# peterbudai/redux

Hardware: AMD Instinct MI355X
Metric: encode MB/s (whole node), per-block bitstream bit-exact (higher is better)
Workload: dtype u32

## Files before the change

### redux_amd/csrc/redux_hip.hip

```cpp
#include "redux_coder.hpp"
#include "redux_any.hpp"
#include "redux_gen.hpp"
#include "redux_encode.hpp"
#include "redux_decode.hpp"
#include "redux_decode_adaptive.hpp"
#include "redux_decode_wave.hpp"
#include "redux_decode_cells.hpp"
#include "redux_pack.hpp"
#include "redux_table.hpp"
#include "redux_coop.hpp"
#include "redux_synth.hpp"
#include "redux_static.hpp"
#include "redux_planes.hpp"
#include "redux_delta.hpp"
#include "redux_base.hpp"
#include "redux_hist.hpp"
#include "redux_plane_static.hpp"
#include "redux_segment_static.hpp"
#include "redux_context_static.hpp"
#include "redux_crc.hpp"
#include "redux_store.hpp"
#include "redux_const.hpp"
#include "redux_cost.hpp"

// ... 38 lines not shown
    const int st = any::compress_stream(P, a.trees + blk * a.tree_words, a.in + o0, len, a.slots + blk * a.slot_bytes,
                                        a.slot_cap, bi, bo);
    a.sizes[blk]  = (uint32_t)bo;
    a.status[blk] = st;
}

struct AnyDecArgs {
    const uint8_t  *in;
    const uint64_t *in_offsets;
    uint64_t        nblocks;
    uint8_t        *out;
    uint32_t       *out_sizes;
    int32_t        *status;
    uint64_t       *in_used;
    uint32_t       *trees;
    uint64_t        tree_words;
    uint32_t        block_size;
    uint32_t        sb, fb, cb;
};

__global__ void __launch_bounds__(64) k_decode_any(AnyDecArgs a)
{
    const uint64_t blk = (uint64_t)blockIdx.x * 64 + threadIdx.x;
    if (blk >= a.nblocks)
        return;
    const uint64_t o0 = a.in_offsets[blk], o1 = a.in_offsets[blk + 1];
    const any::Params P = any::make_params(a.sb, a.fb, a.cb);
    uint64_t  bi, bo;
    const int st = any::decompress_stream(P, a.trees + blk * a.tree_words, a.in + o0, o1 - o0,
                                          a.out + blk * (uint64_t)a.block_size, a.block_size, bi, bo);
    a.out_sizes[blk] = (uint32_t)bo;
    a.status[blk]    = st;
    if (a.in_used)
        a.in_used[blk] = bi;
}

static inline uint64_t align_up(uint64_t v, uint64_t a) { return (v + a - 1) / a * a; }

struct Geometry {
    uint64_t nblocks;
    uint64_t slot_bytes;
    uint32_t slot_cap;
    uint32_t rc_n;
    uint32_t nfreeze;
    bool     u16, fixup;
    bool     any;
    bool     gen;
    uint64_t tree_bytes;
    bool     coop;
    bool     coop_linear;
    uint32_t pair_width;
    uint32_t coop_win;
    uint32_t coop_nwin;
    uint64_t off_rc, off_sizes, off_mode, off_slots, off_trees, off_table, off_seen, off_cstate, off_pairs, total;
};

static int check_params(const redux_params *p)
{
    if (!p)
        return REDUX_INVALID_INPUT;
    const int st = redux_params_check(p->symbol_bits, p->freq_bits, p->code_bits);
    if (st != REDUX_OK)
        return st;
    if (p->symbol_bits > 16)
        return REDUX_UNSUPPORTED;
    return REDUX_OK;
}

static bool is_any(const redux_params *p) { return p->symbol_bits != 8 || p->code_bits > 32; }
static uint64_t gen_updates(const redux_params *p, uint32_t block_size)
{
    const uint64_t nsym    = (uint64_t)block_size * 8 / p->symbol_bits;
    const uint64_t nfreeze = ((1ull << p->freq_bits) - 1) - ((1ull << p->symbol_bits) + 1);
    return nsym < nfreeze ? nsym : nfreeze;
}
static bool gen_decode_cells(const redux_params *p, uint32_t block_size)
{
    if (p->symbol_bits >= 8)
        return gen_updates(p, block_size) + (1ull << (p->symbol_bits - 1)) <= 65535;
    return true;
}
static bool gen_needs_fixup(const redux_params *p, uint32_t block_size)
{
    return p->symbol_bits < 8 && (1ull << p->symbol_bits) + 1 + gen_updates(p, block_size) > (1ull << 17) + 64;
}
static bool is_gen(const redux_params *p, uint32_t block_size)
{
    if (p->code_bits > 32 || p->symbol_bits == 8 || p->symbol_bits > 12 || block_size > (1u << 22))
        return false;
    return gen_decode_cells(p, block_size);
}
static bool gen_decode_in_workspace(const redux_params *p, uint64_t nblocks)
{
    (void)nblocks;
    return p->symbol_bits >= 11;
}
static uint64_t gen_decode_tree_bytes(const redux_params *p) { return (1ull << (p->symbol_bits - 4)) * 32; }
static bool cells8_takes(const redux_params *p, uint32_t block_size, uint64_t nslots, bool table)
{
    return p->symbol_bits == 8 && p->code_bits <= 32 && block_size > 65536 && block_size <= (1u << 22) &&
           (nslots == 0 || nslots > kWaveDecMaxBlocks || (nslots > kWaveDecManyBlocks && block_size >= kWaveDecLargeBlock)) && !table;
}
static uint32_t cells8_rc_entries(const redux_params *p, uint32_t block_size)
{
    const uint64_t nfreeze = ((1ull << p->freq_bits) - 1) - 257;
    return (uint32_t)((block_size < nfreeze ? block_size : nfreeze) + 1 + 32);
}
static bool cells8_needs_fixup(const redux_params *p, uint32_t block_size)
{
    return 257ull + cells8_rc_entries(p, block_size) - 33 > (1ull << 17) + 64;
}

static uint64_t slot_cap_for(const redux_params *p, uint32_t block_size)
{
    const uint64_t freq_max = (1ull << p->freq_bits) - 1;
    if (is_any(p)) {
        const uint64_t K = (1ull << p->symbol_bits) + 1;
        const uint64_t n = (uint64_t)block_size * 8 / p->symbol_bits + 1;
        uint32_t       lg = 0;
        while ((1ull << lg) < K + n)
            lg++;
        const uint64_t per = (lg < p->freq_bits ? lg : p->freq_bits) + 2;
        return n * per / 8 + p->code_bits / 8 + 64;
    }
    const uint64_t n        = block_size;
    const bool     freezes  = 257ull + n > freq_max;
    const uint64_t bits     = freezes ? n * (p->freq_bits + 2) : n * 9;
    return bits / 8 + 1024;
}

static Geometry geometry(const redux_params *p, uint64_t in_len, uint32_t block_size, bool static_model = false, bool allow_coop = true)
{
    Geometry g;
    memset(&g, 0, sizeof g);
    g.nblocks = in_len == 0 ? 1 : (in_len + block_size - 1) / block_size;
    const uint64_t cap = static_model ? ((uint64_t)block_size + 1) * (p->freq_bits + 2) / 8 + 1024 : slot_cap_for(p, block_size);
    g.slot_cap   = cap > 0xFFFFFF00ull ? 0xFFFFFF00u : (uint32_t)cap;
    g.slot_bytes = align_up((uint64_t)g.slot_cap + 32, 128);
    if (((g.slot_bytes / 128) & 1) == 0)
        g.slot_bytes += 128;
    const uint64_t freq_max = (1ull << p->freq_bits) - 1;
    g.nfreeze = (uint32_t)(freq_max - 257);
    const uint64_t maxlen = in_len < block_size ? in_len : block_size;
    g.rc_n  = (uint32_t)((maxlen < g.nfreeze ? maxlen : g.nfreeze) + 1);
    g.u16   = block_size <= 65536;
    g.fixup = (257ull + (uint64_t)(g.rc_n - 1)) >= (1ull << 17);
    g.rc_n += 32;
    g.any = !static_model && is_any(p);
    if (static_model)
        g.rc_n = 0;
    g.gen = !static_model && is_gen(p, block_size) && 64ull * g.slot_bytes < (1ull << 32);
    if (g.gen) {
        const uint64_t k0      = (1ull << p->symbol_bits) + 1;
        const uint64_t nsym    = maxlen * 8 / p->symbol_bits;
        const uint64_t nfreeze = freq_max - k0;
        g.any     = false;
        g.nfreeze = (uint32_t)(nfreeze < 0xFFFFFFFFull ? nfreeze : 0xFFFFFFFFull);
        g.rc_n    = (uint32_t)((nsym < nfreeze ? nsym : nfreeze) + 1 + 32);
        g.u16     = false;
        g.fixup   = true;
        g.tree_bytes = 0;
    }
    if (g.any) {
        g.rc_n       = 0;
        g.u16        = false;
        g.fixup      = true;
        g.tree_bytes = align_up(((1ull << p->symbol_bits) + 2) * 4, 256);
    }
    g.pair_width = g.u16 ? 64u : 1u;
    const uint64_t lanes_total = g.u16 ? (g.nblocks + 63) / 64 * 64 : g.nblocks;
    g.coop_win  = block_size + 1;
    g.coop_nwin = 1;
    if (!g.u16) {
        uint64_t w = kCoopWindowBytes / 2 / (8 * lanes_total);
        w = w > kCoopWindowMax ? kCoopWindowMax : w;
        w = w < 4096 ? 4096 : w;
        if (w < (uint64_t)block_size + 1) {
            g.coop_nwin = (uint32_t)(((uint64_t)block_size + 1 + w - 1) / w);
            g.coop_win  = (uint32_t)((((uint64_t)block_size + 1 + g.coop_nwin - 1) / g.coop_nwin + 31) & ~31ull);
        }
    }
    const uint64_t pair_bytes = (g.u16 ? lanes_total * ((uint64_t)g.coop_win + kCoopSlack) : 2 * lanes_total * coop_block_pitch(g.coop_win)) * 8;
    const bool linear = g.nblocks < 64 && !g.u16;
    g.coop = allow_coop && !static_model && !g.any && !g.gen && g.nblocks <= (g.u16 ? kCoopMaxBlocks : kCoopMaxLargeBlocks) && block_size >= kCoopMinBlock &&
             (linear ? g.nblocks : 64ull) * g.slot_bytes < (1ull << 32) && pair_bytes <= (g.u16 ? kCoopMaxPairBytes : kCoopWindowBytes + (64ull << 20));
    if (g.coop)
        g.rc_n = g.u16 ? g.coop_win + 64 : 2 * ((g.coop_win + 64 + 31) & ~31u);
    g.coop_linear = g.coop && linear;
    g.off_rc    = 0;
    g.off_sizes = align_up(g.off_rc + (uint64_t)g.rc_n * 8, 256);
    g.off_mode  = align_up(g.off_sizes + g.nblocks * 4, 256);
    g.off_slots = g.off_mode + 256 + kClaimWords * 4;
    const bool     one_each = g.coop_linear || (!g.any && !g.gen && !static_model && !g.coop && 64ull * g.slot_bytes >= (1ull << 32));
    const uint64_t nslots = one_each ? g.nblocks : (g.nblocks + 63) / 64 * 64 + 1;
    g.off_trees = align_up(g.off_slots + nslots * g.slot_bytes + (g.nblocks + 63) / 64 * 128, 256);
    g.off_table = align_up(g.off_trees + (g.gen ? (g.nblocks + 63) / 64 * 64 : g.nblocks) * g.tree_bytes, 256);
    g.off_seen  = g.off_table + align_up(g.nblocks * sizeof(redux_block), 256);
    g.off_cstate = g.off_seen + align_up(table_seen_words(g.nblocks) * 4, 256);
    g.off_pairs  = g.off_cstate + ((g.coop && !g.u16) ? align_up(g.nblocks * (8 + 256) * 4, 256) : 0);
    g.total = g.off_pairs + (g.coop ? pair_bytes : 0);
    return g;
}

static Geometry geometry_ws(const redux_params *p, uint64_t in_len, uint32_t block_size, uint64_t workspace_bytes)
{
    Geometry g = geometry(p, in_len, block_size);
    if (g.coop && workspace_bytes < g.total)
        g = geometry(p, in_len, block_size, false, false);
    return g;
}

#define HIP_TRY(expr)                                                                                  \
    do {                                                                                               \
        hipError_t e_ = (expr);                                                                        \
        if (e_ != hipSuccess) {                                                                        \
            fprintf(stderr, "redux_hip: %s failed: %s (%s:%d)\n", #expr, hipGetErrorString(e_),       \
                    __FILE__, __LINE__);                                                               \
            return REDUX_IO_ERROR;                                                                     \
        }                                                                                              \
    } while (0)

static uint32_t cu_count()
{
    static std::atomic<int> cus[16];
    int dev = 0;
    if (hipGetDevice(&dev) != hipSuccess || dev < 0 || dev >= 16)
        return 256;
    int n = cus[dev].load(std::memory_order_relaxed);
    if (n == 0) {
        if (hipDeviceGetAttribute(&n, hipDeviceAttributeMultiprocessorCount, dev) != hipSuccess || n <= 0)
            n = 256;
        cus[dev].store(n, std::memory_order_relaxed);
    }
    return (uint32_t)n;
}

enum class EncKernel { PairCb32, Pair, SingleU16, SingleU32, Gen, GenPair, Any, CoopCb32, Coop };
enum class DecKernel { LockCb32, Lock, GenericU16, GenericU32, Cells, CellsFixup, CellsWorkspace, Cells8, Cells8Fixup, Any, Wave, WaveFixup };

static uint32_t encode_lanes(const Geometry &g, uint32_t block_size)
{
    return (64ull * g.slot_bytes < (1ull << 32) && 64ull * block_size < (1ull << 32)) ? 64u : 1u;
}

static EncKernel pick_encode_kernel(const Geometry &g, const redux_params *p, bool aligned16, uint32_t block_size)
{
    if (g.gen)
        return p->symbol_bits < 8 ? EncKernel::Gen : EncKernel::GenPair;
    if (g.any)
        return EncKernel::Any;
    bool coop = g.coop;
#ifdef REDUX_AB
    if (getenv("REDUX_ENCODE_KERNEL"))
        coop = false;
#endif
    if (coop)
        return p->code_bits == 32 ? EncKernel::CoopCb32 : EncKernel::Coop;
    bool pair = g.u16 && aligned16 && encode_lanes(g, block_size) == 64;
#ifdef REDUX_AB
    const char *force = getenv("REDUX_ENCODE_KERNEL");
    if (force && !strcmp(force, "single"))
        pair = false;
#endif
    if (pair)
        return p->code_bits == 32 ? EncKernel::PairCb32 : EncKernel::Pair;
    return g.u16 ? EncKernel::SingleU16 : EncKernel::SingleU32;
}

static Geometry decode_geometry(const redux_params *p, uint32_t block_size) { return geometry(p, block_size, block_size, false, false); }

static DecKernel pick_decode_kernel(const Geometry &g, const redux_params *p, uint64_t nslots, uint32_t block_size, bool table)
{
    if (g.gen) {
        if (gen_needs_fixup(p, block_size))
            return DecKernel::CellsFixup;
        return gen_decode_in_workspace(p, nslots ? nslots : ~0ull) ? DecKernel::CellsWorkspace : DecKernel::Cells;
    }
    if (g.any)
        return DecKernel::Any;
    if (cells8_takes(p, block_size, nslots, table))
        return cells8_needs_fixup(p, block_size) ? DecKernel::Cells8Fixup : DecKernel::Cells8;
    bool wave = nslots != 0 && nslots <= kWaveDecMaxBlocks && !(g.u16 && !g.fixup);
#ifdef REDUX_AB
    if (getenv("REDUX_DECODE_KERNEL"))
        wave = false;
#endif
    if (wave)
        return g.fixup ? DecKernel::WaveFixup : DecKernel::Wave;
    bool lock = g.u16 && !g.fixup;
#ifdef REDUX_AB
    if (getenv("REDUX_DECODE_KERNEL"))
        lock = false;
#endif
    if (lock)
        return p->code_bits == 32 ? DecKernel::LockCb32 : DecKernel::Lock;
    return g.u16 ? DecKernel::GenericU16 : DecKernel::GenericU32;
}

}

#include "redux_host.hpp"

using namespace redux;

static host::EncodeCoder adaptive_encoder(const redux_params *p, uint32_t block_size)
{
    return {[=](uint64_t max_in, bool several, uint64_t &ws, uint64_t &bound) {
                ws    = several ? geometry(p, max_in, block_size, false, false).total : redux_encode_workspace_bytes(p, max_in, block_size);
                bound = redux_encode_bound(p, max_in, block_size);
            },
            [=](host::Slot &s, uint64_t len, uint64_t bound, void *ws, uint64_t ws_bytes, hipStream_t st) {
                return redux_encode_blocks_dev(p, s.d_in.p, len, block_size, s.d_out.p, bound, s.d_off.p, s.d_st.p, s.d_sum.p, ws,
                                               ws_bytes, st);
            }};
}

static host::EncodeCoder static_encoder(const redux_params *p, const uint32_t *cum, uint32_t block_size)
{
    return {[=](uint64_t max_in, bool, uint64_t &ws, uint64_t &bound) {
// ... 396 lines not shown
}

uint64_t redux_encode_bound(const redux_params *p, uint64_t in_len, uint32_t block_size)
{
    if (check_params(p) != REDUX_OK || block_size == 0)
        return 0;
    const Geometry g = geometry(p, in_len, block_size);
    return g.nblocks * (uint64_t)g.slot_cap;
}

uint64_t redux_encode_workspace_bytes(const redux_params *p, uint64_t in_len, uint32_t block_size)
{
    if (check_params(p) != REDUX_OK || block_size == 0)
        return 0;
    return geometry(p, in_len, block_size).total;
}

static int encode_slots_impl(const redux_params *p, const void *d_in, uint64_t in_len, uint32_t block_size,
                             const redux_block *d_table, uint64_t tbl_blocks, bool tbl_aligned16, void *d_block_status,
                             void *d_workspace, uint64_t workspace_bytes, void *stream, uint64_t nblocks_real = 0)
{
    int st = check_params(p);
    if (st != REDUX_OK)
        return st;
    if (block_size == 0 || !d_workspace || !d_block_status || (in_len && !d_in))
        return REDUX_INVALID_INPUT;
    const Geometry g = geometry_ws(p, d_table ? tbl_blocks * (uint64_t)block_size : in_len, block_size, workspace_bytes);
    if (d_table && (g.gen || g.any || in_len > 0xFFFFFFFFull || tbl_blocks == 0))
        return tbl_blocks == 0 ? REDUX_INVALID_INPUT : REDUX_UNSUPPORTED;
    if (workspace_bytes < g.total)
        return REDUX_OUTPUT_TOO_SMALL;
    if (((uintptr_t)d_workspace) & 255)
        return REDUX_INVALID_INPUT;
    hipStream_t s  = (hipStream_t)stream;
    uint8_t    *ws = (uint8_t *)d_workspace;

    if (d_table) {
        TableCheckArgs ta;
        ta.in         = d_table;
        ta.out        = (redux_block *)(ws + g.off_table);
        ta.nentries   = tbl_blocks;
        ta.nblocks    = nblocks_real;
        ta.bytes      = in_len;
        ta.block_size = block_size;
        ta.aligned16  = tbl_aligned16 ? 1u : 0u;
        ta.seen       = (uint32_t *)(ws + g.off_seen);
        ta.sizes      = (uint32_t *)(ws + g.off_sizes);
        ta.status     = (int32_t *)d_block_status;
        const uint64_t n0 = std::max(nblocks_real, table_seen_words(nblocks_real));
        k_table_prepare<<<(uint32_t)((n0 + 255) / 256), 256, 0, s>>>(ta);
        k_table_check<<<(uint32_t)((tbl_blocks + 255) / 256), 256, 0, s>>>(ta);
        d_table = ta.out;
    }
    HIP_TRY(hipMemsetAsync(ws + g.off_mode, 0, 256 + kClaimWords * 4, s));
    if (g.gen) {
        GenEncArgs ga;
        ga.in         = (const uint8_t *)d_in;
        ga.in_len     = in_len;
        ga.nblocks    = g.nblocks;
        ga.slots      = ws + g.off_slots;
        ga.slot_bytes = g.slot_bytes;
        ga.sizes      = (uint32_t *)(ws + g.off_sizes);
        ga.status     = (int32_t *)d_block_status;
        ga.rc         = (const double *)(ws + g.off_rc);
        ga.block_size = block_size;
        ga.slot_cap   = g.slot_cap;
        ga.nfreeze    = g.nfreeze;
        ga.code_bits  = p->code_bits;
        k_fill_rc_from<<<(g.rc_n + 255) / 256, 256, 0, s>>>((double *)(ws + g.off_rc), g.rc_n, (1u << p->symbol_bits) + 1u);
        const uint32_t grid64 = (uint32_t)((g.nblocks + 63) / 64);
        switch (p->symbol_bits) {
#define REDUX_GEN_ENC(SB) case SB: k_encode_gen<SB><<<grid64, 64, 0, s>>>(ga); break;
#define REDUX_GEN_ENC_PAIR(SB)                                                                                         \
    case SB: k_encode_gen_pair<SB><<<(uint32_t)((g.nblocks + GenTree<SB>::kBlocks - 1) / GenTree<SB>::kBlocks), 256, 0, s>>>(ga); break;
            REDUX_GEN_ENC(1) REDUX_GEN_ENC(2) REDUX_GEN_ENC(3) REDUX_GEN_ENC(4) REDUX_GEN_ENC(5) REDUX_GEN_ENC(6) REDUX_GEN_ENC(7)
            REDUX_GEN_ENC_PAIR(9) REDUX_GEN_ENC_PAIR(10) REDUX_GEN_ENC_PAIR(11) REDUX_GEN_ENC_PAIR(12)
#undef REDUX_GEN_ENC
#undef REDUX_GEN_ENC_PAIR
        default: return REDUX_UNSUPPORTED;
        }
        HIP_TRY(hipGetLastError());
        return REDUX_OK;
    }
    if (g.any) {
        AnyEncArgs aa;
        aa.in         = (const uint8_t *)d_in;
        aa.in_len     = in_len;
        aa.nblocks    = g.nblocks;
        aa.slots      = ws + g.off_slots;
        aa.slot_bytes = g.slot_bytes;
        aa.sizes      = (uint32_t *)(ws + g.off_sizes);
        aa.status     = (int32_t *)d_block_status;
        aa.trees      = (uint32_t *)(ws + g.off_trees);
        aa.tree_words = g.tree_bytes / 4;
        aa.block_size = block_size;
        aa.slot_cap   = g.slot_cap;
        aa.sb = p->symbol_bits; aa.fb = p->freq_bits; aa.cb = p->code_bits;
        k_encode_any<<<(uint32_t)((g.nblocks + 63) / 64), 64, 0, s>>>(aa);
        HIP_TRY(hipGetLastError());
        return REDUX_OK;
    }

    k_fill_rc<<<(g.rc_n + 255) / 256, 256, 0, s>>>((double *)(ws + g.off_rc), g.rc_n);

    EncArgs a;
    a.in         = (const uint8_t *)d_in;
    a.in_len     = in_len;
    a.nblocks    = g.nblocks;
    a.slots      = ws + g.off_slots;
    a.slot_bytes = g.slot_bytes;
    a.sizes      = (uint32_t *)(ws + g.off_sizes);
    a.status     = (int32_t *)d_block_status;
    a.rc         = (const double *)(ws + g.off_rc);
    a.block_size = block_size;
    a.slot_cap   = g.slot_cap;
    a.nfreeze    = g.nfreeze;
    a.code_bits  = p->code_bits;
    a.aligned16  = ((((uintptr_t)d_in) & 15) == 0 && (d_table ? tbl_aligned16 : (block_size & 15) == 0)) ? 1 : 0;
    a.claims     = (uint32_t *)(ws + g.off_mode + 256);
    a.table      = d_table;
    a.pair_width = g.pair_width;
    a.win0 = 0; a.winlen = block_size + 1; a.rc_frozen = 0.0; a.cstate = nullptr; a.cbase = nullptr;
    a.lanes = encode_lanes(g, block_size);
    const uint32_t grid = (uint32_t)((g.nblocks + a.lanes - 1) / a.lanes);
    const EncKernel which = pick_encode_kernel(g, p, a.aligned16 != 0, block_size);
    if (which == EncKernel::PairCb32 || which == EncKernel::Pair || which == EncKernel::CoopCb32 || which == EncKernel::Coop)
        HIP_TRY(hipMemsetAsync(ws + g.off_mode, g.coop_linear ? 2 : (1 | 2), 4, s));
    switch (which) {
    case EncKernel::CoopCb32:
    case EncKernel::Coop: {
        uint2         *pairs = (uint2 *)(ws + g.off_pairs);
        const uint32_t cgrid = (uint32_t)((g.nblocks + 63) / 64);
        const bool     cb32  = which == EncKernel::CoopCb32;
        {
            const double r = 1.0 / (double)(257ull + g.nfreeze);
            uint64_t     u;
            memcpy(&u, &r, 8);
            u += 4;
            memcpy(&a.rc_frozen, &u, 8);
        }
        a.winlen = g.coop_win;
        a.cstate = !g.u16 ? (uint32_t *)(ws + g.off_cstate) : nullptr;
        a.cbase  = a.cstate ? a.cstate + g.nblocks * 8 : nullptr;
        if (g.u16) {
            k_coop_model<false><<<(uint32_t)g.nblocks, 64, 0, s>>>(a, pairs);
            if (g.fixup) {
                if (cb32) k_coop_chain<true, true><<<cgrid, 128, 0, s>>>(a, pairs);
                else      k_coop_chain<false, true><<<cgrid, 128, 0, s>>>(a, pairs);
            } else {
                if (cb32) k_coop_chain<true, false><<<cgrid, 128, 0, s>>>(a, pairs);
                else      k_coop_chain<false, false><<<cgrid, 128, 0, s>>>(a, pairs);
            }
            break;
        }
        const uint64_t longest = d_table ? block_size : (in_len < block_size ? in_len : block_size);
        const uint32_t rc_half = g.rc_n / 2;
        const uint64_t pair_half = g.nblocks * coop_block_pitch(g.coop_win);
        double        *rcs[2] = {(double *)(ws + g.off_rc), (double *)(ws + g.off_rc) + rc_half};
        uint2         *prs[2] = {pairs, pairs + pair_half};
        k_coop_model<true><<<(uint32_t)g.nblocks, 64, 0, s>>>(a, prs[0]);
        for (uint32_t w = 0; w < g.coop_nwin && (uint64_t)w * g.coop_win <= longest; w++) {
            EncArgs ac = a, am = a;
            ac.win0 = w * g.coop_win;
            ac.rc   = rcs[w & 1];
            am.win0 = (w + 1) * g.coop_win;
            if (w)
                k_fill_rc_from<<<(rc_half + 255) / 256, 256, 0, s>>>(rcs[w & 1], rc_half, 257u + ac.win0);
            const bool more = w + 1 < g.coop_nwin && (uint64_t)am.win0 <= longest;
            const uint2 *pc = prs[w & 1];
            uint2       *pm = prs[(w + 1) & 1];
            const uint32_t sgrid = cgrid + (uint32_t)g.nblocks;
#define REDUX_COOP_LAUNCH(CB, FX, LIN)                                                                                 \
    do {                                                                                                               \
        if (more) k_coop_step<CB, FX, LIN><<<sgrid, 128, 0, s>>>(ac, am, pc, pm, cgrid);                               \
        else      k_coop_chain<CB, FX, LIN, true><<<cgrid, 128, 0, s>>>(ac, pc);                                       \
    } while (0)
            if (g.coop_linear) {
                if (g.fixup) { if (cb32) REDUX_COOP_LAUNCH(true, true, true); else REDUX_COOP_LAUNCH(false, true, true); }
                else         { if (cb32) REDUX_COOP_LAUNCH(true, false, true); else REDUX_COOP_LAUNCH(false, false, true); }
            } else {
                if (g.fixup) { if (cb32) REDUX_COOP_LAUNCH(true, true, false); else REDUX_COOP_LAUNCH(false, true, false); }
                else         { if (cb32) REDUX_COOP_LAUNCH(true, false, false); else REDUX_COOP_LAUNCH(false, false, false); }
            }
#undef REDUX_COOP_LAUNCH
        }
        break;
    }
    case EncKernel::PairCb32: k_encode_pair<false, true><<<grid, 128, 0, s>>>(a); break;
    case EncKernel::Pair: k_encode_pair<false, false><<<grid, 128, 0, s>>>(a); break;
    case EncKernel::SingleU16: k_encode<true, false><<<grid, 64, 0, s>>>(a); break;
    case EncKernel::SingleU32: k_encode<false, true><<<grid, 64, 0, s>>>(a); break;
    case EncKernel::Gen:
    case EncKernel::GenPair:
    case EncKernel::Any: break;
    }
    HIP_TRY(hipGetLastError());
    return REDUX_OK;
}

int redux_encode_slots_dev(const redux_params *p, const void *d_in, uint64_t in_len, uint32_t block_size,
                           void *d_block_status, void *d_workspace, uint64_t workspace_bytes, void *stream)
{
    return encode_slots_impl(p, d_in, in_len, block_size, nullptr, 0, false, d_block_status, d_workspace, workspace_bytes, stream);
}

static int compact_with(const Geometry &g, void *d_out, uint64_t out_cap, void *d_out_offsets, void *d_block_status,
                        void *d_summary, void *d_workspace, uint64_t workspace_bytes, void *stream,
                        const redux_block *d_table = nullptr, uint64_t nblocks_real = 0, const uint8_t *d_stored = nullptr,
                        const void *d_raw = nullptr, uint32_t block_size = 0)
{
    if (!d_workspace || !d_block_status || !d_out_offsets || !d_out)
        return REDUX_INVALID_INPUT;
    if (workspace_bytes < g.off_pairs)
        return REDUX_OUTPUT_TOO_SMALL;
    hipStream_t s  = (hipStream_t)stream;
    uint8_t    *ws = (uint8_t *)d_workspace;

    ScanArgs sa;
    sa.sizes   = (const uint32_t *)(ws + g.off_sizes);
    sa.status  = (const int32_t *)d_block_status;
    sa.offsets = (uint64_t *)d_out_offsets;
    sa.summary = (int32_t *)d_summary;
    sa.nblocks = d_table ? nblocks_real : g.nblocks;
    if (scan_is_coalesced(sa))
        k_scan_sizes_coalesced<<<1, 1024, 0, s>>>(sa);
    else
        k_scan_sizes<<<1, 1024, 0, s>>>(sa);

    CompactArgs ca;
    ca.slots      = ws + g.off_slots;
    ca.slot_bytes = g.slot_bytes;
    ca.offsets    = (const uint64_t *)d_out_offsets;
    ca.out        = (uint8_t *)d_out;
    ca.out_cap    = out_cap;
    ca.status     = (int32_t *)d_block_status;
    ca.summary    = (int32_t *)d_summary;
    ca.nblocks    = g.nblocks;
    ca.mode       = (const uint32_t *)(ws + g.off_mode);
    ca.cap_rows   = (uint32_t)(g.slot_bytes / 4);
    ca.table      = d_table;
    ca.stored     = d_stored;
    ca.raw        = (const uint8_t *)d_raw;
    ca.block_size = block_size;
    k_compact<<<(uint32_t)g.nblocks, 256, 0, s>>>(ca);
    if (!g.any && !g.gen && (g.u16 || g.coop)) {
        const uint32_t tiles = (ca.cap_rows + kTileRows - 1) / kTileRows + 1;
        const uint32_t groups = (uint32_t)((g.nblocks + 63) / 64);
        k_compact_rows<<<(groups + 7) / 8 * 8 * tiles, 256, 0, s>>>(ca);
    }
    HIP_TRY(hipGetLastError());
    return REDUX_OK;
}

int redux_compact_slots_dev(const redux_params *p, uint64_t in_len, uint32_t block_size, void *d_out,
                            uint64_t out_cap, void *d_out_offsets, void *d_block_status, void *d_summary,
                            void *d_workspace, uint64_t workspace_bytes, void *stream)
{
    int st = check_params(p);
    if (st != REDUX_OK)
        return st;
    if (block_size == 0)
        return REDUX_INVALID_INPUT;
    return compact_with(geometry_ws(p, in_len, block_size, workspace_bytes), d_out, out_cap, d_out_offsets, d_block_status, d_summary,
                        d_workspace, workspace_bytes, stream);
}

int redux_encode_blocks_dev(const redux_params *p, const void *d_in, uint64_t in_len, uint32_t block_size,
                            void *d_out, uint64_t out_cap, void *d_out_offsets, void *d_block_status,
                            void *d_summary, void *d_workspace, uint64_t workspace_bytes, void *stream)
{
    int st = redux_encode_slots_dev(p, d_in, in_len, block_size, d_block_status, d_workspace, workspace_bytes, stream);
    if (st != REDUX_OK)
        return st;
    return redux_compact_slots_dev(p, in_len, block_size, d_out, out_cap, d_out_offsets, d_block_status, d_summary,
                                   d_workspace, workspace_bytes, stream);
}

int redux_encode_blocks_v_dev(const redux_params *p, const void *d_in, uint64_t in_bytes, const void *d_table,
                              uint64_t nentries, uint64_t nblocks, uint32_t block_size, uint32_t flags, void *d_out,
                              uint64_t out_cap, void *d_out_offsets, void *d_block_status, void *d_summary, void *d_workspace,
                              uint64_t workspace_bytes, void *stream)
{
    if (!d_table || nblocks == 0 || nentries < nblocks)
        return REDUX_INVALID_INPUT;
    if (nentries > 0xFFFFFFF0ull || nblocks > 0xFFFFFFF0ull || !d_block_status || !d_workspace)
        return REDUX_INVALID_INPUT;
    int st = encode_slots_impl(p, d_in, in_bytes, block_size, (const redux_block *)d_table, nentries,
                               (flags & REDUX_V_ALIGNED16) != 0, d_block_status, d_workspace, workspace_bytes, stream, nblocks);
    if (st != REDUX_OK)
        return st;
    const Geometry g = geometry_ws(p, nentries * (uint64_t)block_size, block_size, workspace_bytes);
    st = compact_with(g, d_out, out_cap, d_out_offsets, d_block_status, d_summary, d_workspace, workspace_bytes, stream,
                      (const redux_block *)((uint8_t *)d_workspace + g.off_table), nblocks);
    if (st != REDUX_OK)
        return st;
    k_table_verdict<<<1, 1, 0, (hipStream_t)stream>>>((const uint32_t *)((uint8_t *)d_workspace + g.off_seen) + table_seen_words(nblocks) - 1,
                                                      (int32_t *)d_summary);
    HIP_TRY(hipGetLastError());
    return REDUX_OK;
}
// ... 2671 lines not shown
```

### redux_amd/csrc/redux_pack.hpp

```cpp
#pragma once

#include "redux_coder.hpp"
#include "redux_encode.hpp"
#include "redux_store.hpp"

#include "../../include/redux_hip.h"

#include <hip/hip_runtime.h>
#include <stdint.h>

namespace redux {

__global__ void k_summarize(const int32_t *status, uint64_t nblocks, int32_t *summary)
{
    uint32_t bad = 0;
    uint64_t first = ~0ull;
    for (uint64_t b = (uint64_t)blockIdx.x * blockDim.x + threadIdx.x; b < nblocks; b += (uint64_t)gridDim.x * blockDim.x)
        if (status[b] != REDUX_OK) {
            bad++;
            if (first == ~0ull)
                first = b;
        }
    if (bad) {
        atomicAdd(&summary[1], (int32_t)bad);
        atomicCAS(&summary[0], REDUX_OK, status[first]);
    }
}

struct ScanArgs {
    const uint32_t *sizes;
    const int32_t  *status;
    uint64_t       *offsets;
    int32_t        *summary;
    uint64_t        nblocks;
};

static inline bool scan_is_coalesced(const ScanArgs &a)
{
    return a.nblocks % 4096 == 0 && a.nblocks / 4096 <= 16 &&
           ((((uintptr_t)a.sizes) | ((uintptr_t)a.status) | ((uintptr_t)a.offsets)) & 15) == 0;
}

__global__ void __launch_bounds__(1024) k_scan_sizes_coalesced(ScanArgs a)
{
    __shared__ uint32_t bad_cnt;
    __shared__ uint64_t bad_first;
    __shared__ uint64_t wtot[2][16];
    const uint32_t tid = threadIdx.x;
    if (tid == 0) {
        bad_cnt   = 0;
        bad_first = ~0ull;
    }
    const uint32_t nch  = (uint32_t)(a.nblocks / 4096);
    const uint32_t lane = tid & 63, wave = tid >> 6;
    const uint4   *s4   = reinterpret_cast<const uint4 *>(a.sizes);
    const int4    *t4   = reinterpret_cast<const int4 *>(a.status);
    uint32_t stp[16];
    {
        int4 stv[16];
#pragma unroll
        for (int i = 0; i < 16; i++)
            stv[i] = (uint32_t)i < nch ? t4[i * 1024 + tid] : make_int4(0, 0, 0, 0);
#pragma unroll
        for (int i = 0; i < 16; i++)
            stp[i] = ((uint32_t)stv[i].x & 0xFFu) | (((uint32_t)stv[i].y & 0xFFu) << 8) | (((uint32_t)stv[i].z & 0xFFu) << 16) |
                     ((uint32_t)stv[i].w << 24);
    }
    uint4 sz[16];
#pragma unroll
    for (int i = 0; i < 16; i++)
        sz[i] = (uint32_t)i < nch ? s4[i * 1024 + tid] : make_uint4(0, 0, 0, 0);
    uint64_t running = 0;
    uint32_t nb      = 0;
    uint64_t fb      = ~0ull;
#pragma unroll
    for (int i = 0; i < 16; i++) {
        if ((uint32_t)i >= nch)
            continue;
        const uint32_t qs   = sz[i].x + sz[i].y + sz[i].z + sz[i].w;
        uint32_t       incl = qs;
#pragma unroll
        for (int o = 1; o < 64; o <<= 1) {
            const uint32_t v = __shfl_up(incl, o);
            incl += lane >= (uint32_t)o ? v : 0u;
        }
        if (lane == 63)
            wtot[i & 1][wave] = incl;
        __syncthreads();
        uint64_t before = 0, total = 0;
#pragma unroll
        for (int w = 0; w < 16; w++) {
            const uint64_t v = wtot[i & 1][w];
            before += (uint32_t)w < wave ? v : 0;
            total += v;
        }
        const uint64_t q  = (uint64_t)i * 1024 + tid;
        const uint64_t o0 = running + before + (incl - qs);
        const uint64_t o1 = o0 + sz[i].x, o2 = o1 + sz[i].y, o3 = o2 + sz[i].z;
        ulonglong2    *op = reinterpret_cast<ulonglong2 *>(a.offsets + 4 * q);
        op[0]             = make_ulonglong2(o0, o1);
        op[1]             = make_ulonglong2(o2, o3);
        running += total;
        if (stp[i] != 0) {
#pragma unroll
            for (int k = 0; k < 4; k++) {
                const uint32_t st = (stp[i] >> (8 * k)) & 0xFFu;
                if (st != REDUX_OK) {
                    nb++;
                    const uint64_t cand = ((4 * q + k) << 8) | st;
                    fb                  = cand < fb ? cand : fb;
                }
            }
        }
    }
    if (nb) {
        atomicAdd(&bad_cnt, nb);
        atomicMin((unsigned long long *)&bad_first, (unsigned long long)fb);
    }
    __syncthreads();
    if (tid == 0) {
        a.offsets[a.nblocks] = running;
        if (a.summary) {
            a.summary[0] = bad_cnt ? (int32_t)(bad_first & 0xFF) : REDUX_OK;
            a.summary[1] = (int32_t)bad_cnt;
        }
    }
}

__global__ void __launch_bounds__(1024) k_scan_sizes(ScanArgs a)
{
    __shared__ uint64_t part[1024];
    __shared__ uint32_t bad_cnt;
    __shared__ uint64_t bad_first;
    const uint32_t tid = threadIdx.x;
    if (tid == 0) {
        bad_cnt   = 0;
        bad_first = ~0ull;
    }
    const uint64_t per = (a.nblocks + 1023) / 1024;
    const uint64_t b0  = per * tid < a.nblocks ? per * tid : a.nblocks;
    const uint64_t b1  = b0 + per < a.nblocks ? b0 + per : a.nblocks;
    uint64_t       sum = 0;
    uint32_t       nb  = 0;
    uint64_t       fb  = ~0ull;
    const bool quads = per <= 64 && (per & 3) == 0 && (a.nblocks % per) == 0 &&
                       ((((uintptr_t)a.sizes) | ((uintptr_t)a.status) | ((uintptr_t)a.offsets)) & 15) == 0;
    uint4      sz[16];
    if (quads) {
        const uint4 *s4 = reinterpret_cast<const uint4 *>(a.sizes + b0);
        const int4  *t4 = reinterpret_cast<const int4 *>(a.status + b0);
        int4         stv[16];
#pragma unroll
        for (int i = 0; i < 16; i++) {
            const bool in = b0 + 4 * i < b1;
            sz[i]  = in ? s4[i] : make_uint4(0, 0, 0, 0);
            stv[i] = in ? t4[i] : make_int4(0, 0, 0, 0);
        }
#pragma unroll
        for (int i = 0; i < 16; i++) {
            sum += (uint64_t)sz[i].x + sz[i].y + sz[i].z + sz[i].w;
            const int32_t st4[4] = {stv[i].x, stv[i].y, stv[i].z, stv[i].w};
#pragma unroll
            for (int k = 0; k < 4; k++)
                if (st4[k] != REDUX_OK) {
                    nb++;
                    if (fb == ~0ull)
                        fb = ((b0 + 4 * i + k) << 8) | (uint32_t)st4[k];
                }
        }
    } else {
        for (uint64_t b = b0; b < b1; b++) {
            sum += a.sizes[b];
            const int32_t st = a.status[b];
            if (st != REDUX_OK) {
                nb++;
                if (fb == ~0ull)
                    fb = (b << 8) | (uint32_t)st;
// ... 6 lines not shown
        atomicAdd(&bad_cnt, nb);
        atomicMin((unsigned long long *)&bad_first, (unsigned long long)fb);
    }
    for (uint32_t o = 1; o < 1024; o <<= 1) {
        const uint64_t v = tid >= o ? part[tid - o] : 0;
        __syncthreads();
        part[tid] += v;
        __syncthreads();
    }
    uint64_t run = tid ? part[tid - 1] : 0;
    if (quads) {
        ulonglong2 *o2 = reinterpret_cast<ulonglong2 *>(a.offsets + b0);
#pragma unroll
        for (int i = 0; i < 16; i++)
            if (b0 + 4 * i < b1) {
                const uint64_t r1 = run + sz[i].x, r2 = r1 + sz[i].y, r3 = r2 + sz[i].z;
                o2[2 * i]     = make_ulonglong2(run, r1);
                o2[2 * i + 1] = make_ulonglong2(r2, r3);
                run           = r3 + sz[i].w;
            }
    } else {
        for (uint64_t b = b0; b < b1; b++) {
            a.offsets[b] = run;
            run += a.sizes[b];
        }
    }
    if (tid == 1023)
        a.offsets[a.nblocks] = part[1023];
    if (tid == 0 && a.summary) {
        a.summary[0] = bad_cnt ? (int32_t)(bad_first & 0xFF) : REDUX_OK;
        a.summary[1] = (int32_t)bad_cnt;
    }
}

struct CompactArgs {
    const uint8_t  *slots;
    uint64_t        slot_bytes;
    const uint64_t *offsets;
    uint8_t        *out;
    uint64_t        out_cap;
    int32_t        *status;
    int32_t        *summary;
    uint64_t        nblocks;
    const uint32_t *mode;
    uint32_t        cap_rows;
    const redux_block *table;
    const uint8_t  *stored;
    const uint8_t  *raw;
    uint32_t        block_size;
};

__global__ void __launch_bounds__(256) k_compact(CompactArgs a)
{
    const uint64_t b = blockIdx.x;
    const uint32_t mode = *a.mode;
    if (b >= a.nblocks || ((mode & 1u) && !a.stored))
        return;
    const uint32_t bx  = (mode & 2u) ? 3u : 0u;
    const uint32_t sel = (mode & 2u) ? 0x00010203u : 0x03020100u;
    const uint64_t lb = a.table ? a.table[b].index : b;
    if (lb == kIdleEntry)
        return;
    const bool raw = a.stored && a.stored[lb];
    if ((mode & 1u) && !raw)
        return;
    const uint64_t o0 = a.offsets[lb], o1 = a.offsets[lb + 1];
    const uint32_t tid = threadIdx.x;
    if (o1 > a.out_cap) {
        if (tid == 0) {
            if (a.status[lb] == REDUX_OK)
                a.status[lb] = REDUX_OUTPUT_TOO_SMALL;
            if (a.summary) {
                atomicCAS(&a.summary[0], REDUX_OK, REDUX_OUTPUT_TOO_SMALL);
                atomicAdd(&a.summary[1], 1);
            }
        }
        return;
    }
    const uint32_t n   = (uint32_t)(o1 - o0);
    const uint8_t *src = a.slots + b * a.slot_bytes;
    uint8_t       *dst = a.out + o0;
    if (raw) {
        store_copy(a.raw + lb * a.block_size, dst, n, tid, 256);
        return;
    }

    uint32_t head = (uint32_t)((16 - ((uintptr_t)dst & 15)) & 15);
    if (head > n)
        head = n;
    if (tid < head)
        dst[tid] = src[tid ^ bx];
    const uint32_t nchunks = (n - head) >> 4;
    const uint32_t dq = head >> 2, r = head & 3;
    const uint4   *s16 = reinterpret_cast<const uint4 *>(src);
    uint4         *d16 = reinterpret_cast<uint4 *>(dst + head);
    for (uint32_t i = tid; i < nchunks; i += 256) {
        const uint4    A = s16[i], B = s16[i + 1];
        const uint32_t d[8] = {A.x, A.y, A.z, A.w, B.x, B.y, B.z, B.w};
        uint32_t       v[5];
#pragma unroll
        for (int k = 0; k < 5; k++)
            v[k] = __builtin_amdgcn_perm(0u, dq == 0 ? d[k] : dq == 1 ? d[k + 1] : dq == 2 ? d[k + 2] : d[k + 3], sel);
        uint4 o;
        o.x = __builtin_amdgcn_alignbyte(v[1], v[0], r);
        o.y = __builtin_amdgcn_alignbyte(v[2], v[1], r);
        o.z = __builtin_amdgcn_alignbyte(v[3], v[2], r);
        o.w = __builtin_amdgcn_alignbyte(v[4], v[3], r);
        d16[i] = o;
    }
    const uint32_t done = head + (nchunks << 4);
    if (tid < n - done)
        dst[done + tid] = src[(done + tid) ^ bx];
}

constexpr uint32_t kTileRows = 64;
__global__ void __launch_bounds__(256) k_compact_rows(CompactArgs a)
{
    const uint32_t mode = *a.mode;
    if ((mode & 1u) == 0)
        return;
    const uint32_t sel = (mode & 2u) ? 0x00010203u : 0x03020100u;
    __shared__ uint32_t tile[(kTileRows + 1) * 65];
    __shared__ uint64_t s_dst[64];
    __shared__ uint32_t s_n[64], s_sh[64];
    __shared__ uint32_t s_maxj;
    const uint32_t tiles = (a.cap_rows + kTileRows - 1) / kTileRows + 1;
    const uint32_t y   = blockIdx.x >> 3;
    const uint64_t g   = (uint64_t)(y / tiles) * 8 + (blockIdx.x & 7u);
    const uint32_t r0  = (y % tiles) * kTileRows;
    if (g * 64 >= a.nblocks)
        return;
    const uint32_t tid   = threadIdx.x;
    if (tid == 0)
        s_maxj = 0;
    __syncthreads();
    if (tid < 64) {
        const uint64_t b = g * 64 + tid;
        uint64_t       d = 0;
        uint32_t       n = 0, sh = 0;
        const uint64_t lb = b < a.nblocks ? (a.table ? a.table[b].index : b) : kIdleEntry;
        if (lb != kIdleEntry && !(a.stored && a.stored[lb])) {
            const uint64_t o0 = a.offsets[lb], o1 = a.offsets[lb + 1];
            if (o1 <= a.out_cap) {
                n  = (uint32_t)(o1 - o0);
                sh = (uint32_t)((uintptr_t)(a.out + o0) & 3);
                d  = (uint64_t)(uintptr_t)(a.out + o0) - sh;
                atomicMax(&s_maxj, (sh + n + 3) >> 2);
            } else if (r0 == 0) {
                if (a.status[lb] == REDUX_OK)
                    a.status[lb] = REDUX_OUTPUT_TOO_SMALL;
                if (a.summary) {
                    atomicCAS(&a.summary[0], REDUX_OK, REDUX_OUTPUT_TOO_SMALL);
                    atomicAdd(&a.summary[1], 1);
                }
            }
        }
        s_dst[tid] = d;
        s_n[tid]   = n;
        s_sh[tid]  = sh;
    }
    __syncthreads();
    if (r0 >= s_maxj)
        return;
    const uint4 *area = reinterpret_cast<const uint4 *>(a.slots + g * (64 * a.slot_bytes + 128));
    uint4 v[4], lead = make_uint4(0, 0, 0, 0);
// ... 59 lines not shown
```

Measured before the change: 366,400.

## Fuse encode setup kernels, parallelize size scan, skip unneeded compaction launches

Merges the rc-table fill and the mode/claim memset into one prepare kernel, and only issues the memset for gen/any paths. The offset scan moves from a single-block kernel (with a special coalesced case) to a two-pass multi-block chunked scan that stores per-chunk totals in workspace. A slot layout is computed per geometry so that the linear compact kernel is skipped or launched with a capped grid-stride grid when encoders leave slots in row layout. This cuts launch count and idle blocks at the cost of an extra scan pass and some added layout bookkeeping.

Result: no change. 367,900, median of 6 (+0.4%).

```diff
diff --git a/redux_amd/csrc/redux_hip.hip b/redux_amd/csrc/redux_hip.hip
--- a/redux_amd/csrc/redux_hip.hip
+++ b/redux_amd/csrc/redux_hip.hip
@@ -114,6 +114,7 @@
     uint32_t pair_width;
     uint32_t coop_win;
     uint32_t coop_nwin;
+    enum SlotLayout : uint8_t { Linear, Rows, ByInput } layout;
     uint64_t off_rc, off_sizes, off_mode, off_slots, off_trees, off_table, off_seen, off_cstate, off_pairs, total;
 };
 
@@ -172,6 +173,8 @@
 {
     return 257ull + cells8_rc_entries(p, block_size) - 33 > (1ull << 17) + 64;
 }
+
+static Geometry::SlotLayout slot_layout_of(const Geometry &g, const redux_params *p, uint32_t block_size, bool static_model);
 
 static uint64_t slot_cap_for(const redux_params *p, uint32_t block_size)
 {
@@ -260,6 +263,7 @@
     g.off_seen  = g.off_table + align_up(g.nblocks * sizeof(redux_block), 256);
     g.off_cstate = g.off_seen + align_up(table_seen_words(g.nblocks) * 4, 256);
     g.off_pairs  = g.off_cstate + ((g.coop && !g.u16) ? align_up(g.nblocks * (8 + 256) * 4, 256) : 0);
+    g.layout     = slot_layout_of(g, p, block_size, static_model);
     g.total = g.off_pairs + (g.coop ? pair_bytes : 0);
     return g;
 }
@@ -327,6 +331,19 @@
     if (pair)
         return p->code_bits == 32 ? EncKernel::PairCb32 : EncKernel::Pair;
     return g.u16 ? EncKernel::SingleU16 : EncKernel::SingleU32;
+}
+
+static bool leaves_rows(const Geometry &g, EncKernel k)
+{
+    return k == EncKernel::PairCb32 || k == EncKernel::Pair || ((k == EncKernel::CoopCb32 || k == EncKernel::Coop) && !g.coop_linear);
+}
+
+static Geometry::SlotLayout slot_layout_of(const Geometry &g, const redux_params *p, uint32_t block_size, bool static_model)
+{
+    if (static_model)
+        return Geometry::Linear;
+    const bool al = leaves_rows(g, pick_encode_kernel(g, p, true, block_size)), un = leaves_rows(g, pick_encode_kernel(g, p, false, block_size));
+    return al != un ? Geometry::ByInput : al ? Geometry::Rows : Geometry::Linear;
 }
 
 static Geometry decode_geometry(const redux_params *p, uint32_t block_size) { return geometry(p, block_size, block_size, false, false); }
@@ -829,7 +846,8 @@
         k_table_check<<<(uint32_t)((tbl_blocks + 255) / 256), 256, 0, s>>>(ta);
         d_table = ta.out;
     }
-    HIP_TRY(hipMemsetAsync(ws + g.off_mode, 0, 256 + kClaimWords * 4, s));
+    if (g.gen || g.any)
+        HIP_TRY(hipMemsetAsync(ws + g.off_mode, 0, 256 + kClaimWords * 4, s));
     if (g.gen) {
         GenEncArgs ga;
         ga.in         = (const uint8_t *)d_in;
@@ -878,8 +896,6 @@
         return REDUX_OK;
     }
 
-    k_fill_rc<<<(g.rc_n + 255) / 256, 256, 0, s>>>((double *)(ws + g.off_rc), g.rc_n);
-
     EncArgs a;
     a.in         = (const uint8_t *)d_in;
     a.in_len     = in_len;
@@ -901,8 +917,13 @@
     a.lanes = encode_lanes(g, block_size);
     const uint32_t grid = (uint32_t)((g.nblocks + a.lanes - 1) / a.lanes);
     const EncKernel which = pick_encode_kernel(g, p, a.aligned16 != 0, block_size);
-    if (which == EncKernel::PairCb32 || which == EncKernel::Pair || which == EncKernel::CoopCb32 || which == EncKernel::Coop)
-        HIP_TRY(hipMemsetAsync(ws + g.off_mode, g.coop_linear ? 2 : (1 | 2), 4, s));
+    const bool     swapped = which == EncKernel::PairCb32 || which == EncKernel::Pair || which == EncKernel::CoopCb32 || which == EncKernel::Coop;
+    const bool     rows    = leaves_rows(g, which);
+    if (g.layout != Geometry::ByInput && rows != (g.layout == Geometry::Rows))
+        return REDUX_UNSUPPORTED;
+    const uint32_t mode_words = (256 + kClaimWords * 4) / 4;
+    k_prepare_encode<<<(std::max(g.rc_n, mode_words) + 255) / 256, 256, 0, s>>>((double *)(ws + g.off_rc), g.rc_n, (uint32_t *)(ws + g.off_mode),
+                                                                             mode_words, swapped ? (rows ? 0x03030303u : 0x02020202u) : 0u);
     switch (which) {
     case EncKernel::CoopCb32:
     case EncKernel::Coop: {
@@ -993,16 +1014,21 @@
     hipStream_t s  = (hipStream_t)stream;
     uint8_t    *ws = (uint8_t *)d_workspace;
 
+    const bool may_rows = g.layout != Geometry::Linear, may_linear = g.layout != Geometry::Rows;
     ScanArgs sa;
     sa.sizes   = (const uint32_t *)(ws + g.off_sizes);
-    sa.status  = (const int32_t *)d_block_status;
+    sa.status  = (int32_t *)d_block_status;
     sa.offsets = (uint64_t *)d_out_offsets;
     sa.summary = (int32_t *)d_summary;
     sa.nblocks = d_table ? nblocks_real : g.nblocks;
-    if (scan_is_coalesced(sa))
-        k_scan_sizes_coalesced<<<1, 1024, 0, s>>>(sa);
-    else
+    sa.chunks  = (ScanChunk *)(ws + g.off_seen);
+    if (!d_table && scan_is_parallel(sa)) {
+        const uint32_t nch = (uint32_t)((sa.nblocks + kScanChunk - 1) / kScanChunk);
+        k_scan_totals<<<nch, 256, 0, s>>>(sa);
+        k_scan_chunks<<<nch, 256, 0, s>>>(sa);
+    } else {
         k_scan_sizes<<<1, 1024, 0, s>>>(sa);
+    }
 
     CompactArgs ca;
     ca.slots      = ws + g.off_slots;
@@ -1019,10 +1045,14 @@
     ca.stored     = d_stored;
     ca.raw        = (const uint8_t *)d_raw;
     ca.block_size = block_size;
-    k_compact<<<(uint32_t)g.nblocks, 256, 0, s>>>(ca);
-    if (!g.any && !g.gen && (g.u16 || g.coop)) {
+    if (may_linear || d_stored) {
+        const bool     whole = g.layout == Geometry::Linear || d_stored;
+        const uint64_t grid  = whole ? g.nblocks : std::min<uint64_t>(g.nblocks, 16ull * cu_count());
+        k_compact<<<(uint32_t)grid, 256, 0, s>>>(ca);
+    }
+    if (may_rows) {
+        const uint32_t groups = (uint32_t)((g.nblocks + 63) / 64);
         const uint32_t tiles = (ca.cap_rows + kTileRows - 1) / kTileRows + 1;
-        const uint32_t groups = (uint32_t)((g.nblocks + 63) / 64);
         k_compact_rows<<<(groups + 7) / 8 * 8 * tiles, 256, 0, s>>>(ca);
     }
     HIP_TRY(hipGetLastError());
diff --git a/redux_amd/csrc/redux_pack.hpp b/redux_amd/csrc/redux_pack.hpp
--- a/redux_amd/csrc/redux_pack.hpp
+++ b/redux_amd/csrc/redux_pack.hpp
@@ -27,102 +27,178 @@
     }
 }
 
+__global__ void __launch_bounds__(256) k_prepare_encode(double *rc, uint32_t n, uint32_t *mode_area, uint32_t words, uint32_t mode)
+{
+    const uint32_t i = blockIdx.x * blockDim.x + threadIdx.x;
+    if (i < n) {
+        const double r = 1.0 / (double)(257u + i);
+        rc[i] = __longlong_as_double(__double_as_longlong(r) + 4);
+    }
+    if (i < words)
+        mode_area[i] = i == 0 ? mode : 0u;
+}
+
+struct ScanChunk {
+    uint64_t total;
+    uint64_t bad_first;
+    uint32_t bad_cnt;
+    uint32_t pad[3];
+};
+constexpr uint32_t kScanChunk     = 1024;
+constexpr uint32_t kScanMaxChunks = 1024;
+
 struct ScanArgs {
     const uint32_t *sizes;
-    const int32_t  *status;
+    int32_t        *status;
     uint64_t       *offsets;
     int32_t        *summary;
     uint64_t        nblocks;
+    ScanChunk      *chunks;
 };
 
-static inline bool scan_is_coalesced(const ScanArgs &a)
-{
-    return a.nblocks % 4096 == 0 && a.nblocks / 4096 <= 16 &&
+static inline bool scan_is_parallel(const ScanArgs &a)
+{
+    return (a.nblocks + kScanChunk - 1) / kScanChunk <= kScanMaxChunks &&
            ((((uintptr_t)a.sizes) | ((uintptr_t)a.status) | ((uintptr_t)a.offsets)) & 15) == 0;
 }
 
-__global__ void __launch_bounds__(1024) k_scan_sizes_coalesced(ScanArgs a)
-{
-    __shared__ uint32_t bad_cnt;
-    __shared__ uint64_t bad_first;
-    __shared__ uint64_t wtot[2][16];
-    const uint32_t tid = threadIdx.x;
+__device__ __forceinline__ uint4 scan_quad(const uint32_t *p, uint64_t b, uint64_t n)
+{
+    if (b + 4 <= n)
+        return *reinterpret_cast<const uint4 *>(p + b);
+    uint4 v = make_uint4(0, 0, 0, 0);
+    if (b < n) v.x = p[b];
+    if (b + 1 < n) v.y = p[b + 1];
+    if (b + 2 < n) v.z = p[b + 2];
+    return v;
+}
+
+__device__ __forceinline__ void mark_too_small(int32_t *status, int32_t *summary, uint64_t lb)
+{
+    if (status[lb] == REDUX_OK)
+        status[lb] = REDUX_OUTPUT_TOO_SMALL;
+    if (summary) {
+        atomicCAS(&summary[0], REDUX_OK, REDUX_OUTPUT_TOO_SMALL);
+        atomicAdd(&summary[1], 1);
+    }
+}
+
+__global__ void __launch_bounds__(256) k_scan_totals(ScanArgs a)
+{
+    __shared__ uint64_t w_sum[4], w_first[4];
+    __shared__ uint32_t w_cnt[4];
+    const uint32_t tid = threadIdx.x, lane = tid & 63, wave = tid >> 6;
+    const uint64_t b   = ((uint64_t)blockIdx.x * 256 + tid) * 4;
+    const uint4    sz  = scan_quad(a.sizes, b, a.nblocks);
+    const uint4    st  = scan_quad(reinterpret_cast<const uint32_t *>(a.status), b, a.nblocks);
+    uint64_t       sum = (uint64_t)sz.x + sz.y + sz.z + sz.w;
+    uint32_t       cnt = 0;
+    uint64_t       fb  = ~0ull;
+    if ((st.x | st.y | st.z | st.w) != 0) {
+        const uint32_t s4[4] = {st.x, st.y, st.z, st.w};
+#pragma unroll
+        for (int k = 3; k >= 0; k--)
+            if (s4[k] != REDUX_OK) {
+                cnt++;
+                fb = ((b + k) << 8) | (s4[k] & 0xFFu);
+            }
+    }
+#pragma unroll
+    for (int o = 32; o; o >>= 1) {
+        sum += __shfl_xor(sum, o);
+        cnt += __shfl_xor(cnt, o);
+        const uint64_t f = __shfl_xor(fb, o);
+        fb               = f < fb ? f : fb;
+    }
+    if (lane == 0) {
+        w_sum[wave]   = sum;
+        w_cnt[wave]   = cnt;
+        w_first[wave] = fb;
+    }
+    __syncthreads();
     if (tid == 0) {
-        bad_cnt   = 0;
-        bad_first = ~0ull;
-    }
-    const uint32_t nch  = (uint32_t)(a.nblocks / 4096);
-    const uint32_t lane = tid & 63, wave = tid >> 6;
-    const uint4   *s4   = reinterpret_cast<const uint4 *>(a.sizes);
-    const int4    *t4   = reinterpret_cast<const int4 *>(a.status);
-    uint32_t stp[16];
-    {
-        int4 stv[16];
-#pragma unroll
-        for (int i = 0; i < 16; i++)
-            stv[i] = (uint32_t)i < nch ? t4[i * 1024 + tid] : make_int4(0, 0, 0, 0);
-#pragma unroll
-        for (int i = 0; i < 16; i++)
-            stp[i] = ((uint32_t)stv[i].x & 0xFFu) | (((uint32_t)stv[i].y & 0xFFu) << 8) | (((uint32_t)stv[i].z & 0xFFu) << 16) |
-                     ((uint32_t)stv[i].w << 24);
-    }
-    uint4 sz[16];
-#pragma unroll
-    for (int i = 0; i < 16; i++)
-        sz[i] = (uint32_t)i < nch ? s4[i * 1024 + tid] : make_uint4(0, 0, 0, 0);
-    uint64_t running = 0;
-    uint32_t nb      = 0;
-    uint64_t fb      = ~0ull;
-#pragma unroll
-    for (int i = 0; i < 16; i++) {
-        if ((uint32_t)i >= nch)
-            continue;
-        const uint32_t qs   = sz[i].x + sz[i].y + sz[i].z + sz[i].w;
-        uint32_t       incl = qs;
-#pragma unroll
-        for (int o = 1; o < 64; o <<= 1) {
-            const uint32_t v = __shfl_up(incl, o);
-            incl += lane >= (uint32_t)o ? v : 0u;
-        }
-        if (lane == 63)
-            wtot[i & 1][wave] = incl;
-        __syncthreads();
-        uint64_t before = 0, total = 0;
-#pragma unroll
-        for (int w = 0; w < 16; w++) {
-            const uint64_t v = wtot[i & 1][w];
-            before += (uint32_t)w < wave ? v : 0;
-            total += v;
-        }
-        const uint64_t q  = (uint64_t)i * 1024 + tid;
-        const uint64_t o0 = running + before + (incl - qs);
-        const uint64_t o1 = o0 + sz[i].x, o2 = o1 + sz[i].y, o3 = o2 + sz[i].z;
-        ulonglong2    *op = reinterpret_cast<ulonglong2 *>(a.offsets + 4 * q);
-        op[0]             = make_ulonglong2(o0, o1);
-        op[1]             = make_ulonglong2(o2, o3);
-        running += total;
-        if (stp[i] != 0) {
-#pragma unroll
-            for (int k = 0; k < 4; k++) {
-                const uint32_t st = (stp[i] >> (8 * k)) & 0xFFu;
-                if (st != REDUX_OK) {
-                    nb++;
-                    const uint64_t cand = ((4 * q + k) << 8) | st;
-                    fb                  = cand < fb ? cand : fb;
-                }
-            }
-        }
-    }
-    if (nb) {
-        atomicAdd(&bad_cnt, nb);
-        atomicMin((unsigned long long *)&bad_first, (unsigned long long)fb);
-    }
-    __syncthreads();
-    if (tid == 0) {
-        a.offsets[a.nblocks] = running;
-        if (a.summary) {
-            a.summary[0] = bad_cnt ? (int32_t)(bad_first & 0xFF) : REDUX_OK;
-            a.summary[1] = (int32_t)bad_cnt;
+        ScanChunk c;
+        c.total     = w_sum[0] + w_sum[1] + w_sum[2] + w_sum[3];
+        c.bad_cnt   = w_cnt[0] + w_cnt[1] + w_cnt[2] + w_cnt[3];
+        c.bad_first = w_first[0];
+        for (int w = 1; w < 4; w++)
+            c.bad_first = w_first[w] < c.bad_first ? w_first[w] : c.bad_first;
+        c.pad[0] = c.pad[1] = c.pad[2] = 0;
+        a.chunks[blockIdx.x] = c;
+        if (blockIdx.x == 0 && a.summary) {
+            a.summary[0] = REDUX_OK;
+            a.summary[1] = 0;
+        }
+    }
+}
+
+__global__ void __launch_bounds__(256) k_scan_chunks(ScanArgs a)
+{
+    __shared__ uint64_t w_base[4], w_quad[4], w_first[4];
+    __shared__ uint32_t w_cnt[4];
+    const uint32_t tid = threadIdx.x, lane = tid & 63, wave = tid >> 6;
+    const uint32_t c = blockIdx.x, nch = gridDim.x;
+    const uint64_t b = ((uint64_t)c * 256 + tid) * 4;
+    const uint4    sz = scan_quad(a.sizes, b, a.nblocks);
+    uint64_t       base = 0;
+    for (uint32_t i = tid; i < c; i += 256)
+        base += a.chunks[i].total;
+    uint32_t cnt = 0;
+    uint64_t fb  = ~0ull;
+    if (c == 0)
+        for (uint32_t i = tid; i < nch; i += 256) {
+            const ScanChunk k = a.chunks[i];
+            cnt += k.bad_cnt;
+            fb = k.bad_first < fb ? k.bad_first : fb;
+        }
+    const uint64_t qs   = (uint64_t)sz.x + sz.y + sz.z + sz.w;
+    uint64_t       incl = qs;
+#pragma unroll
+    for (int o = 1; o < 64; o <<= 1) {
+        const uint64_t v = __shfl_up(incl, o);
+        incl += lane >= (uint32_t)o ? v : 0ull;
+    }
+#pragma unroll
+    for (int o = 32; o; o >>= 1) {
+        base += __shfl_xor(base, o);
+        cnt += __shfl_xor(cnt, o);
+        const uint64_t f = __shfl_xor(fb, o);
+        fb               = f < fb ? f : fb;
+    }
+    if (lane == 63)
+        w_quad[wave] = incl;
+    if (lane == 0) {
+        w_base[wave]  = base;
+        w_cnt[wave]   = cnt;
+        w_first[wave] = fb;
+    }
+    __syncthreads();
+    uint64_t o0 = incl - qs;
+#pragma unroll
+    for (uint32_t w = 0; w < 4; w++) {
+        o0 += w_base[w];
+        o0 += w < wave ? w_quad[w] : 0ull;
+    }
+    const uint64_t o1 = o0 + sz.x, o2 = o1 + sz.y, o3 = o2 + sz.z, o4 = o3 + sz.w;
+    if (b + 4 <= a.nblocks) {
+        ulonglong2 *op = reinterpret_cast<ulonglong2 *>(a.offsets + b);
+        op[0]          = make_ulonglong2(o0, o1);
+        op[1]          = make_ulonglong2(o2, o3);
+    } else {
+        if (b < a.nblocks) a.offsets[b] = o0;
+        if (b + 1 < a.nblocks) a.offsets[b + 1] = o1;
+        if (b + 2 < a.nblocks) a.offsets[b + 2] = o2;
+    }
+    if (b < a.nblocks && b + 4 >= a.nblocks)
+        a.offsets[a.nblocks] = o4;
+    if (c == 0 && tid == 0 && a.summary) {
+        const uint32_t n = w_cnt[0] + w_cnt[1] + w_cnt[2] + w_cnt[3];
+        uint64_t       f = w_first[0];
+        for (int w = 1; w < 4; w++)
+            f = w_first[w] < f ? w_first[w] : f;
+        if (n) {
+            a.summary[0] = (int32_t)(f & 0xFF);
+            a.summary[1] = (int32_t)n;
         }
     }
 }
@@ -235,65 +311,60 @@
 
 __global__ void __launch_bounds__(256) k_compact(CompactArgs a)
 {
-    const uint64_t b = blockIdx.x;
     const uint32_t mode = *a.mode;
-    if (b >= a.nblocks || ((mode & 1u) && !a.stored))
+    if ((mode & 1u) && !a.stored)
         return;
     const uint32_t bx  = (mode & 2u) ? 3u : 0u;
     const uint32_t sel = (mode & 2u) ? 0x00010203u : 0x03020100u;
-    const uint64_t lb = a.table ? a.table[b].index : b;
-    if (lb == kIdleEntry)
-        return;
-    const bool raw = a.stored && a.stored[lb];
-    if ((mode & 1u) && !raw)
-        return;
-    const uint64_t o0 = a.offsets[lb], o1 = a.offsets[lb + 1];
     const uint32_t tid = threadIdx.x;
-    if (o1 > a.out_cap) {
-        if (tid == 0) {
-            if (a.status[lb] == REDUX_OK)
-                a.status[lb] = REDUX_OUTPUT_TOO_SMALL;
-            if (a.summary) {
-                atomicCAS(&a.summary[0], REDUX_OK, REDUX_OUTPUT_TOO_SMALL);
-                atomicAdd(&a.summary[1], 1);
-            }
-        }
-        return;
-    }
-    const uint32_t n   = (uint32_t)(o1 - o0);
-    const uint8_t *src = a.slots + b * a.slot_bytes;
-    uint8_t       *dst = a.out + o0;
-    if (raw) {
-        store_copy(a.raw + lb * a.block_size, dst, n, tid, 256);
-        return;
-    }
-
-    uint32_t head = (uint32_t)((16 - ((uintptr_t)dst & 15)) & 15);
-    if (head > n)
-        head = n;
-    if (tid < head)
-        dst[tid] = src[tid ^ bx];
-    const uint32_t nchunks = (n - head) >> 4;
-    const uint32_t dq = head >> 2, r = head & 3;
-    const uint4   *s16 = reinterpret_cast<const uint4 *>(src);
-    uint4         *d16 = reinterpret_cast<uint4 *>(dst + head);
-    for (uint32_t i = tid; i < nchunks; i += 256) {
-        const uint4    A = s16[i], B = s16[i + 1];
-        const uint32_t d[8] = {A.x, A.y, A.z, A.w, B.x, B.y, B.z, B.w};
-        uint32_t       v[5];
-#pragma unroll
-        for (int k = 0; k < 5; k++)
-            v[k] = __builtin_amdgcn_perm(0u, dq == 0 ? d[k] : dq == 1 ? d[k + 1] : dq == 2 ? d[k + 2] : d[k + 3], sel);
-        uint4 o;
-        o.x = __builtin_amdgcn_alignbyte(v[1], v[0], r);
-        o.y = __builtin_amdgcn_alignbyte(v[2], v[1], r);
-        o.z = __builtin_amdgcn_alignbyte(v[3], v[2], r);
-        o.w = __builtin_amdgcn_alignbyte(v[4], v[3], r);
-        d16[i] = o;
-    }
-    const uint32_t done = head + (nchunks << 4);
-    if (tid < n - done)
-        dst[done + tid] = src[(done + tid) ^ bx];
+    for (uint64_t b = blockIdx.x; b < a.nblocks; b += gridDim.x) {
+        const uint64_t lb = a.table ? a.table[b].index : b;
+        if (lb == kIdleEntry)
+            continue;
+        const bool raw = a.stored && a.stored[lb];
+        if ((mode & 1u) && !raw)
+            continue;
+        const uint64_t o0 = a.offsets[lb], o1 = a.offsets[lb + 1];
+        if (o1 > a.out_cap) {
+            if (tid == 0)
+                mark_too_small(a.status, a.summary, lb);
+            continue;
+        }
+        const uint32_t n   = (uint32_t)(o1 - o0);
+        const uint8_t *src = a.slots + b * a.slot_bytes;
+        uint8_t       *dst = a.out + o0;
+        if (raw) {
+            store_copy(a.raw + lb * a.block_size, dst, n, tid, 256);
+            continue;
+        }
+
+        uint32_t head = (uint32_t)((16 - ((uintptr_t)dst & 15)) & 15);
+        if (head > n)
+            head = n;
+        if (tid < head)
+            dst[tid] = src[tid ^ bx];
+        const uint32_t nchunks = (n - head) >> 4;
+        const uint32_t dq = head >> 2, r = head & 3;
+        const uint4   *s16 = reinterpret_cast<const uint4 *>(src);
+        uint4         *d16 = reinterpret_cast<uint4 *>(dst + head);
+        for (uint32_t i = tid; i < nchunks; i += 256) {
+            const uint4    A = s16[i], B = s16[i + 1];
+            const uint32_t d[8] = {A.x, A.y, A.z, A.w, B.x, B.y, B.z, B.w};
+            uint32_t       v[5];
+#pragma unroll
+            for (int k = 0; k < 5; k++)
+                v[k] = __builtin_amdgcn_perm(0u, dq == 0 ? d[k] : dq == 1 ? d[k + 1] : dq == 2 ? d[k + 2] : d[k + 3], sel);
+            uint4 o;
+            o.x = __builtin_amdgcn_alignbyte(v[1], v[0], r);
+            o.y = __builtin_amdgcn_alignbyte(v[2], v[1], r);
+            o.z = __builtin_amdgcn_alignbyte(v[3], v[2], r);
+            o.w = __builtin_amdgcn_alignbyte(v[4], v[3], r);
+            d16[i] = o;
+        }
+        const uint32_t done = head + (nchunks << 4);
+        if (tid < n - done)
+            dst[done + tid] = src[(done + tid) ^ bx];
+    }
 }
 
 constexpr uint32_t kTileRows = 64;
```
